# UMEssen/Body-and-Organ-Analysis

Measured on AMD Instinct MI355X. Metric: CT volumes/sec (512^3 @1.5 mm, total+bca) on MI355X, higher is better.
Workload: dtype f16

## Files before the change

### body-and-organ-analysis_amd/boa_hip/_lib.py

```python
from __future__ import annotations

import ctypes as C
import os

_HERE = os.path.dirname(os.path.abspath(__file__))
LIB_PATH = os.environ.get("BOA_HIP_LIB") or os.path.join(_HERE, "libboa_hip.so")

BOA_OK, BOA_EINVAL, BOA_EHIP, BOA_ENOMEM, BOA_EINF = 0, -1, -2, -3, -4
BOA_DEFLATE_DYNAMIC = 1
BOA_INF_INFO_WORDS, BOA_INF_MS_WORDS = 8, 8
BOA_INF_STATUS = ("ok", "truncated", "invalid", "far", "overrun", "size", "crc", "repair", "trailing")
BOA_PLAN_WORDS = 32
K_CONV_MFMA, K_CONV_FIRST, K_CONVT, K_NORM_FINALIZE, K_HEAD_ACCUM, K_ARGMAX, K_OTHER, K_AGG, K_MORPH, K_RESAMPLE, K_COPY, K_COUNT = range(12)
K_NAMES = ["conv_mfma", "conv_first", "convT_mfma", "norm_finalize", "head_accum", "finalize_argmax", "other", "aggregation",
           "morphology", "resample", "copy_remap"]
CNT_NAMES = ["head_mfma", "head_valu", "conv_ws", "conv_simple", "first_mfma", "first_valu", "f32", "conv_x3", "x3", "head_gather",
             "copy_t", "bbox_vec", "finalize_vec8"]
MAX_STAGES = 8


class NetDesc(C.Structure):
    _fields_ = [
        ("n_stages", C.c_int), ("in_channels", C.c_int), ("num_classes", C.c_int),
        ("features", C.c_int * MAX_STAGES), ("kernel", (C.c_int * 3) * MAX_STAGES),
        ("stride", (C.c_int * 3) * MAX_STAGES), ("n_conv_enc", C.c_int * MAX_STAGES),
        ("n_conv_dec", C.c_int * MAX_STAGES), ("patch", C.c_int * 3), ("norm_eps", C.c_float),
        ("lrelu_slope", C.c_float),
    ]


class BoaError(RuntimeError):
    pass


_lib = None

vp, i32, u64, f32 = C.c_void_p, C.c_int, C.c_size_t, C.c_float
ip = C.POINTER(C.c_int)

_PROTOS = {
    "boa_last_error": (C.c_char_p, []),
    "boa_version": (i32, []),
    "boa_init": (i32, [i32, vp, C.POINTER(vp)]),
    "boa_destroy": (None, [vp]),
    "boa_device_info": (i32, [vp, C.c_char_p, i32, ip, C.POINTER(u64), C.POINTER(u64)]),
    "boa_malloc": (i32, [vp, u64, C.POINTER(vp)]),
    "boa_free": (i32, [vp, vp]),
    "boa_trim": (i32, [vp]),
    "boa_bind_thread": (i32, [vp]),
    "boa_host_alloc": (i32, [vp, C.c_size_t, C.POINTER(vp)]),
    "boa_host_free": (i32, [vp, vp]),
    "boa_mfma_peak": (i32, [vp, i32, i32, C.POINTER(C.c_double)]),
    "boa_memset": (i32, [vp, vp, i32, u64]),
    "boa_h2d": (i32, [vp, vp, vp, u64]),
    "boa_d2h": (i32, [vp, vp, vp, u64]),
    "boa_sync": (i32, [vp]),
    "boa_timer_start": (i32, [vp, i32]),
    "boa_timer_stop": (i32, [vp, i32, C.POINTER(f32)]),
    "boa_prof_enable": (i32, [vp, i32]),
    "boa_prof_reset": (i32, [vp]),
    "boa_prof_get": (i32, [vp, i32, C.POINTER(C.c_double), C.POINTER(C.c_longlong), C.POINTER(C.c_double),
                           C.POINTER(C.c_double)]),
    "boa_debug_counter": (C.c_longlong, [vp, i32, i32]),
    "boa_net_debug_activation": (i32, [vp, i32, i32, i32, i32, vp, ip, ip]),
    "boa_net_debug_layer": (i32, [vp, i32, i32, i32, i32, vp, vp, vp, ip, ip, ip]),
    "boa_head_tile": (i32, [vp, vp, vp, i32, ip, i32, vp, vp, f32, vp, vp, vp, vp, ip, ip]),
    "boa_head_tile_f32": (i32, [vp, i32, vp, u64, vp, i32, ip, i32, vp, vp, f32, vp, vp, vp, vp, ip, ip]),
    "boa_ct_normalize": (i32, [vp, vp, i32, vp, u64, f32, f32, f32, f32]),
    "boa_accumulate_tile": (i32, [vp, vp, vp, vp, vp, i32, ip, ip, ip]),
    "boa_finalize_labels": (i32, [vp, vp, vp, i32, ip, vp, i32, i32, i32, vp, i32, vp, ip, ip, vp]),
    "boa_finalize_labels_planes": (i32, [vp, vp, vp, i32, ip, vp, i32, i32, i32, vp, i32, vp, ip, ip, vp, i32, i32]),
    "boa_net_predict_sliding_window_deferred": (i32, [vp, vp, ip, ip, ip, ip, i32, vp, vp, vp, ip, C.POINTER(vp)]),
    "boa_net_apply_deferred": (i32, [vp, vp, vp, vp, vp, ip]),
    "boa_stash_destroy": (None, [vp]),
    "boa_net_create": (i32, [vp, C.POINTER(NetDesc), vp, u64, i32, i32, C.POINTER(vp)]),
    "boa_net_destroy": (None, [vp]),
    "boa_net_weight_count": (u64, [C.POINTER(NetDesc)]),
    "boa_net_load_weights": (i32, [vp, vp, u64]),
    "boa_net_set_mirroring": (i32, [vp, i32]),
    "boa_net_forward": (i32, [vp, vp, ip, ip, i32, vp]),
    "boa_net_predict_sliding_window": (i32, [vp, vp, ip, ip, ip, ip, i32, vp, vp, vp]),
    "boa_net_labels_supported": (i32, [vp, ip, i32]),
    "boa_net_predict_labels_fold": (i32, [vp, vp, ip, ip, ip, ip, i32, vp, vp, i32, i32, vp, i32, vp, ip, ip, vp]),
    "boa_conv_block_test": (i32, [vp, vp, i32, i32, ip, vp, vp, vp, vp, i32, ip, ip, i32, i32, vp]),
    "boa_convtranspose_test": (i32, [vp, vp, i32, i32, ip, vp, vp, i32, ip, vp]),
    "boa_conv_plan": (i32, [i32, i32, ip, i32, ip, ip, i32, i32, ip, ip]),
    "boa_convt_plan": (i32, [i32, ip, i32, ip, i32, i32, i32, ip]),
    "boa_conv_layer_test": (i32, [vp, i32, i32, ip, vp, i32, vp, vp, vp, i32, vp, vp, vp, vp, vp, vp, i32, ip, ip, ip, vp, vp, vp, vp, ip]),
    "boa_convt_layer_test": (i32, [vp, i32, i32, ip, vp, i32, vp, vp, vp, vp, i32, ip, vp, ip]),
    "boa_tissue_aggregate": (i32, [vp, vp, vp, vp, vp, vp, i32, i32, i32, vp, vp]),
    "boa_slice_label_presence": (i32, [vp, vp, i32, i32, i32, vp]),
    "boa_tissue_projections": (i32, [vp, vp, vp, i32, i32, i32, vp, i32, vp, vp, vp, vp]),
    "boa_label_hu_histogram": (i32, [vp, vp, vp, vp, u64, i32, i32, vp]),
    "boa_label_hu_mask": (i32, [vp, vp, vp, vp, i32, i32, i32, u64, vp]),
    "boa_label_basic_stats": (i32, [vp, vp, i32, vp, ip, i32, vp]),
    "boa_label_apply_lut": (i32, [vp, vp, u64, vp, vp]),
    "boa_group_stats_f64": (i32, [vp, vp, vp, u64, vp, i32, vp, vp]),
    "boa_label_hu_mask_f64": (i32, [vp, vp, vp, vp, i32, C.c_double, C.c_double, u64, vp]),
    "boa_tissue_aggregate_f64": (i32, [vp, vp, vp, vp, vp, vp, i32, i32, i32, vp, vp]),
    "boa_binary_erode": (i32, [vp, vp, vp, vp, i32, i32, i32, i32]),
    "boa_ccl26": (i32, [vp, vp, i32, i32, i32, vp, vp, ip]),
    "boa_ccl_filter_largest": (i32, [vp, vp, vp, u64, vp, i32]),
    "boa_ccl_remove_small": (i32, [vp, vp, vp, u64, C.c_uint32, vp]),
    "boa_ccl_list_components": (i32, [vp, vp, u64, i32, vp, vp, ip]),
    "boa_scatter_u32": (i32, [vp, vp, vp, vp, i32]),
    "boa_ccl_fill_unmarked": (i32, [vp, vp, vp, u64, C.c_uint32, vp, i32]),
    "boa_label_blobs6": (i32, [vp, vp, i32, i32, i32, vp, vp, ip]),
    "boa_label_blobs_filter": (i32, [vp, vp, vp, u64, vp, C.c_uint32, C.c_uint32, vp]),
    "boa_label_select": (i32, [vp, vp, u64, i32, ip, vp]),
    "boa_fill_holes_2d": (i32, [vp, vp, i32, i32, i32, vp, vp, vp]),
    "boa_binary_dilate_cross": (i32, [vp, vp, vp, vp, i32, i32, i32, i32]),
    "boa_mask_assign": (i32, [vp, vp, u64, i32, i32, vp]),
    "boa_label_overlay": (i32, [vp, vp, u64, vp]),
    "boa_median3_inplane": (i32, [vp, vp, i32, i32, i32, i32, vp]),
    "boa_median3_inplane_f64": (i32, [vp, vp, i32, i32, i32, i32, vp]),
    "boa_bits_words": (u64, [i32, i32, i32]),
    "boa_bits_erode_u8": (i32, [vp, vp, vp, i32, i32, i32, i32, i32]),
    "boa_bits_select": (i32, [vp, vp, i32, i32, i32, vp, i32, vp]),
    "boa_bits_unpack": (i32, [vp, vp, i32, i32, i32, vp]),
    "boa_bits_fill_supported": (i32, [i32, i32]),
    "boa_bits_fill_holes_2d": (i32, [vp, vp, i32, i32, i32, i32, vp]),
    "boa_bits_remove_small": (i32, [vp, vp, i32, i32, i32, i32, C.c_uint32, i32]),
    "boa_bits_filter_largest": (i32, [vp, vp, i32, i32, i32, vp, i32]),
    "boa_bits_assign_labels": (i32, [vp, vp, i32, i32, i32, i32, vp, vp]),
    "boa_copy3": (i32, [vp, vp, i32, C.c_longlong, C.POINTER(C.c_longlong), ip, vp, i32, C.c_longlong, C.POINTER(C.c_longlong)]),
    "boa_nonzero_bbox": (i32, [vp, vp, i32, ip, ip]),
    "boa_resample_cubic": (i32, [vp, vp, i32, ip, vp, i32, ip]),
    "boa_resample_nearest_u8": (i32, [vp, vp, ip, vp, ip]),
    "boa_resample_onehot_u8": (i32, [vp, vp, ip, vp, ip, i32]),
    "boa_resize_skimage_f32": (i32, [vp, vp, ip, vp, ip, i32, i32]),
    "boa_resize_logits_argmax": (i32, [vp, vp, i32, ip, ip, ip, ip, i32, vp, i32, vp]),
    "boa_logits_to_probabilities": (i32, [vp, vp, i32, ip, ip, ip, ip, i32, ip, ip, ip, vp, vp, vp]),
    "boa_comm_available": (i32, []),
    "boa_comm_library": (C.c_char_p, []),
    "boa_comm_unique_id": (i32, [vp]),
    "boa_comm_create": (i32, [vp, i32, i32, vp, C.POINTER(vp)]),
    "boa_comm_destroy": (None, [vp]),
    "boa_comm_wait": (i32, [vp]),
    "boa_comm_exchange": (i32, [vp, i32, C.POINTER(vp), C.POINTER(u64), i32, i32, C.POINTER(vp), C.POINTER(u64), i32]),
    "boa_comm_shift_slab": (i32, [vp, i32, i32, i32, i32, i32, i32, vp, vp, i32, ip, vp]),
    "boa_comm_all_reduce": (i32, [vp, vp, u64, i32]),
    "boa_comm_planes_to_owner": (i32, [vp, vp, i32, ip, i32, ip, ip, ip, i32, ip, ip, ip]),
    "boa_comm_stats": (i32, [vp, C.POINTER(C.c_longlong), C.POINTER(C.c_longlong)]),
    "boa_add_f16_planes": (i32, [vp, vp, vp, vp, i32, ip, i32, i32]),
    "boa_ljpeg_decode": (i32, [vp, vp, u64, i32, ip, i32, ip, i32, ip, i32, C.POINTER(C.c_uint32), vp, ip, i32]),
    "boa_jdct_decode": (i32, [vp, vp, u64, i32, ip, i32, i32, i32, ip, i32, ip, i32, C.POINTER(C.c_uint32), i32,
                        C.POINTER(C.c_uint16), vp, ip, i32]),
    "boa_j2k_decode": (i32, [vp, vp, u64, i32, ip, i32, ip, vp, ip]),
    "boa_rle_decode": (i32, [vp, vp, u64, i32, ip, i32, i32, i32, vp, ip, i32]),
    "boa_jls_decode": (i32, [vp, vp, u64, i32, ip, i32, i32, vp, ip, i32]),
    "boa_deflate_bound": (u64, [u64, u64]),
    "boa_deflate_members": (i32, [vp, vp, u64, u64, i32, vp, u64, C.POINTER(u64), C.POINTER(C.c_uint32)]),
    "boa_deflate_members2": (i32, [vp, vp, u64, u64, i32, i32, i32, vp, u64, C.POINTER(u64), C.POINTER(C.c_uint32)]),
    "boa_label_member_presence": (i32, [vp, vp, u64, u64, C.POINTER(C.c_uint32)]),
    "boa_deflate_label_pairs": (i32, [vp, vp, u64, u64, i32, i32, C.POINTER(C.c_uint8), C.POINTER(C.c_uint32), i32, vp, u64, C.POINTER(u64),
                                      C.POINTER(C.c_uint32)]),
    "boa_inflate_default_chunk": (u64, []),
    "boa_inflate_streams": (i32, [vp, vp, u64, i32, C.POINTER(u64), C.POINTER(u64), C.POINTER(u64), C.POINTER(C.c_uint32), u64, vp, u64, ip,
                                  C.POINTER(u64), C.POINTER(C.c_float)]),
}

EXPORTS = sorted(_PROTOS)


def lib():
    global _lib
    if _lib is not None:
        return _lib
    if not os.path.exists(LIB_PATH):
        raise BoaError(
            f"{LIB_PATH} not found: build it with `make -C body-and-organ-analysis_amd` "
            "(or python -c 'import __graft_entry__ as g; g.build()'). There is no CPU fallback.")
    try:
        import torch
    except Exception:
        pass
    L = C.CDLL(LIB_PATH, mode=C.RTLD_GLOBAL)
    for name, (res, args) in _PROTOS.items():
        fn = getattr(L, name)
        fn.restype = res
        fn.argtypes = args
    _lib = L
    return L


def check(rc: int, what: str = ""):
    if rc == BOA_OK:
        return
    msg = lib().boa_last_error().decode("utf-8", "replace")
    text = f"{what}: {msg}" if what else msg
    if rc == BOA_EINVAL:
        raise ValueError(text)
    if rc == BOA_ENOMEM:
        raise MemoryError(text)
    raise BoaError(text)


def int3(v):
    return (C.c_int * 3)(*[int(x) for x in v])
```

### body-and-organ-analysis_amd/boa_hip/resample.py

```python
from __future__ import annotations

import numpy as np

from ._lib import check, int3
from .device import Context, DeviceBuffer

_IN_DTYPES = {np.dtype(np.int16): 0, np.dtype(np.float32): 1, np.dtype(np.float64): 2, np.dtype(np.int32): 3}


def zoomed_shape(shape, zoom):
    zoom = np.broadcast_to(np.asarray(zoom, dtype=np.float64), (len(shape),))
    return tuple(int(round(n * z)) for n, z in zip(shape, zoom))


def resample_cubic_device(ctx: Context, dev_in: DeviceBuffer, in_dtype, in_shape, out_shape, out_dtype=np.int32):
    code = _IN_DTYPES[np.dtype(in_dtype)]
    oc = {np.dtype(np.int32): 0, np.dtype(np.float64): 1}[np.dtype(out_dtype)]
    n = int(np.prod(out_shape))
    out = DeviceBuffer(ctx, n * np.dtype(out_dtype).itemsize)
    check(ctx.lib.boa_resample_cubic(ctx.h, dev_in.vp, code, int3(in_shape), out.vp, oc, int3(out_shape)),
          "boa_resample_cubic")
    return out


def resample_nearest_device(ctx: Context, dev_in: DeviceBuffer, in_shape, out_shape):
    out = DeviceBuffer(ctx, int(np.prod(out_shape)))
    check(ctx.lib.boa_resample_nearest_u8(ctx.h, dev_in.vp, int3(in_shape), out.vp, int3(out_shape)),
          "boa_resample_nearest_u8")
    return out


REF_TO_MEMORY_AXIS = (2, 0, 1)


def resample_onehot_device(ctx: Context, dev_in: DeviceBuffer, in_shape, out_shape, sep_axis=None):
    out = DeviceBuffer(ctx, int(np.prod(out_shape)))
    ax = -1 if sep_axis is None or int(sep_axis) < 0 else REF_TO_MEMORY_AXIS[int(sep_axis)]
    check(ctx.lib.boa_resample_onehot_u8(ctx.h, dev_in.vp, int3(in_shape), out.vp, int3(out_shape), ax),
          "boa_resample_onehot_u8")
    return out


def resample_img(ctx: Context, img: np.ndarray, zoom=0.5, order: int = 0, out_dtype=None, target_shape=None):
    img = np.asarray(img)
    if img.ndim != 3:
        raise ValueError(f"resample_img: 3-D arrays only, got {img.shape}")
    shape = tuple(int(s) for s in target_shape) if target_shape is not None else zoomed_shape(img.shape, zoom)
    if order == 0:
        if img.dtype != np.uint8:
            if img.min() < 0 or img.max() > 255:
                raise ValueError("resample_img(order=0): label values must fit uint8")
            img = img.astype(np.uint8)
        d = DeviceBuffer(ctx, img.size).upload(img)
        o = resample_nearest_device(ctx, d, img.shape, shape)
        res = o.download(shape, np.uint8)
        d.free(), o.free()
        return res
    if order != 3:
        raise ValueError(f"resample_img: order {order} not supported (the reference uses 0 and 3)")
    if img.dtype not in _IN_DTYPES:
        img = img.astype(np.float64)
    od = np.dtype(np.float64 if out_dtype is None else out_dtype)
    d = DeviceBuffer(ctx, img.nbytes).upload(img)
    o = resample_cubic_device(ctx, d, img.dtype, img.shape, shape, od)
    res = o.download(shape, od)
    d.free(), o.free()
    return res


def change_spacing_array(ctx: Context, data: np.ndarray, img_spacing, new_spacing=1.25, target_shape=None, order=0,
                         dtype=None, remove_negative=False):
    old_shape = np.array(data.shape)
    img_spacing = np.array(img_spacing, dtype=np.float32)
    if target_shape is not None:
        zoom = np.array(target_shape) / old_shape
        new_spacing = img_spacing / zoom
    else:
        if type(new_spacing) is float:
            new_spacing = [new_spacing] * 3
        new_spacing = np.array(new_spacing)
        zoom = img_spacing / new_spacing
    if np.array_equal(img_spacing, new_spacing):
        return data, None
    want_i32 = dtype is not None and np.dtype(dtype) == np.int32 and not remove_negative and order == 3
    new = resample_img(ctx, data, zoom, order, out_dtype=np.int32 if want_i32 else None)
    if remove_negative:
        new[new < 1e-4] = 0
    if dtype is not None:
        new = new.astype(dtype, copy=False)
    return new, zoom


def new_affine(affine: np.ndarray, zoom) -> np.ndarray:
    a = np.copy(affine)
    for i in range(3):
        a[:3, i] = a[:3, i] / zoom[i]
    return a
```

### body-and-organ-analysis_amd/csrc/resample.hip

```cpp
#include <math.h>

#include "common.h"
#include "resample_logits.h"

#define NPAD 12

template <typename T>
__global__ __launch_bounds__(256) void k_pad_edge_f64(const T* __restrict__ in, int X, int Y, int Z,
                                                      double* __restrict__ out) {
    const int PX = X + 2 * NPAD, PY = Y + 2 * NPAD, PZ = Z + 2 * NPAD;
    const size_t n = (size_t)PX * PY * PZ;
    size_t i = (size_t)blockIdx.x * 256 + threadIdx.x;
    if (i >= n) return;
    int x, y, z;
    idx3(i, PY, PZ, x, y, z);
    x -= NPAD; y -= NPAD; z -= NPAD;
    x = min(max(x, 0), X - 1);
    y = min(max(y, 0), Y - 1);
    z = min(max(z, 0), Z - 1);
    out[i] = (double)in[((size_t)x * Y + y) * Z + z];
}

struct SplineConsts {
    double z, gain, z_n, init_scale, tail_scale;
};

__global__ __launch_bounds__(64) void k_spline_filter_axis(double* __restrict__ c, int n, size_t st, int n1, size_t st1,
                                                           int n2, size_t st2, SplineConsts k) {
    const size_t line = (size_t)blockIdx.x * 64 + threadIdx.x;
    if (line >= (size_t)n1 * n2) return;
    double* p = c + (line / n2) * st1 + (line % n2) * st2;
    const double z = k.z;
    const double gain = k.gain;
    for (int i = 0; i < n; ++i) p[i * st] *= gain;
    const double z_n = k.z_n;
    double z_i = z;
    const double c0 = p[0];
    double acc = p[0] + z_n * p[(size_t)(n - 1) * st];
    for (int i = 1; i < n; ++i) {
        acc += z_i * (p[i * st] + z_n * p[(size_t)(n - 1 - i) * st]);
        z_i *= z;
    }
    acc *= k.init_scale;
    acc += c0;
    p[0] = acc;
    for (int i = 1; i < n; ++i) p[i * st] += z * p[(size_t)(i - 1) * st];
    p[(size_t)(n - 1) * st] *= k.tail_scale;
    for (int i = n - 2; i >= 0; --i) p[i * st] = z * (p[(size_t)(i + 1) * st] - p[i * st]);
}

__global__ __launch_bounds__(64) void k_spline_filter_contig(double* __restrict__ c, int n, int n1, size_t st1, int n2, size_t st2,
                                                             SplineConsts k) {
    const size_t line = (size_t)blockIdx.x * 64 + threadIdx.x;
    if (line >= (size_t)n1 * n2) return;
    double* p = c + (line / n2) * st1 + (line % n2) * st2;
    const double z = k.z, gain = k.gain, z_n = k.z_n;
    const int nc = n / 8;
    const double c0 = p[0] * gain;
    double acc = c0 + z_n * (p[n - 1] * gain);
    double z_i = z;
    for (int cb = 0; cb < nc; ++cb) {
        double f[8], b[8];
#pragma unroll
        for (int m = 0; m < 8; ++m) f[m] = p[8 * cb + m];
        const int b0 = n - 8 * cb - 8;
#pragma unroll
        for (int m = 0; m < 8; ++m) b[m] = p[b0 + m];
#pragma unroll
        for (int m = 0; m < 8; ++m) {
            const int i = 8 * cb + m;
            if (i >= 1) {
                acc += z_i * (f[m] * gain + z_n * (b[7 - m] * gain));
                z_i *= z;
            }
        }
    }
    for (int i = max(8 * nc, 1); i < n; ++i) {
        acc += z_i * (p[i] * gain + z_n * (p[n - 1 - i] * gain));
        z_i *= z;
    }
    acc *= k.init_scale;
    acc += c0;
    double prev = acc;
    for (int cb = 0; cb < nc; ++cb) {
        double f[8];
#pragma unroll
        for (int m = 0; m < 8; ++m) f[m] = p[8 * cb + m];
#pragma unroll
        for (int m = 0; m < 8; ++m) {
            if (8 * cb + m >= 1) {
                double s = f[m] * gain;
                s += z * prev;
                prev = s;
            }
            f[m] = prev;
        }
#pragma unroll
        for (int m = 0; m < 8; ++m) p[8 * cb + m] = f[m];
    }
    for (int i = 8 * nc; i < n; ++i) {
        if (i >= 1) {
            double s = p[i] * gain;
            s += z * prev;
            prev = s;
        }
        p[i] = prev;
    }
    double nxt = p[n - 1] * k.tail_scale;
    p[n - 1] = nxt;
    int i = n - 2;
    for (; i >= 0 && ((i + 1) & 7) != 0; --i) {
        nxt = z * (nxt - p[i]);
        p[i] = nxt;
    }
    for (; i >= 7; i -= 8) {
        double f[8];
#pragma unroll
        for (int m = 0; m < 8; ++m) f[m] = p[i - 7 + m];
#pragma unroll
        for (int m = 7; m >= 0; --m) {
            nxt = z * (nxt - f[m]);
            f[m] = nxt;
        }
#pragma unroll
        for (int m = 0; m < 8; ++m) p[i - 7 + m] = f[m];
    }
}

__device__ __forceinline__ void cubic_weights(double cc, int* start, double w[4]) {
    const double fl = floor(cc);
    const double x = cc - fl;
    const double y = x, zz = 1.0 - x;
    w[1] = (y * y * (y - 2.0) * 3.0 + 4.0) / 6.0;
    w[2] = (zz * zz * (zz - 2.0) * 3.0 + 4.0) / 6.0;
    w[0] = zz * zz * zz / 6.0;
    w[3] = 1.0 - w[0] - w[1] - w[2];
    *start = (int)fl - 1;
}

__global__ __launch_bounds__(256) void k_zoom_cubic(const double* __restrict__ coef, int X, int Y, int Z, int OX, int OY,
                                                    int OZ, double zx, double zy, double zz_, int out_mode, void* out) {
    const size_t n = (size_t)OX * OY * OZ;
    size_t i = (size_t)blockIdx.x * 256 + threadIdx.x;
    if (i >= n) return;
    int ox, oy, oz;
    idx3(i, OY, OZ, ox, oy, oz);
    const int PY = Y + 2 * NPAD, PZ = Z + 2 * NPAD;
    double wx[4], wy[4], wz[4];
    int sx, sy, sz;
    cubic_weights((double)ox * zx + NPAD, &sx, wx);
    cubic_weights((double)oy * zy + NPAD, &sy, wy);
    cubic_weights((double)oz * zz_ + NPAD, &sz, wz);
    double t = 0.0;
#pragma unroll
    for (int a = 0; a < 4; ++a)
#pragma unroll
        for (int b = 0; b < 4; ++b) {
            const double* row = coef + ((size_t)(sx + a) * PY + (sy + b)) * PZ + sz;
#pragma unroll
            for (int d = 0; d < 4; ++d) {
                double cf = row[d];
                cf *= wx[a];
                cf *= wy[b];
                cf *= wz[d];
                t += cf;
            }
        }
    if (out_mode == 0)
        ((int*)out)[i] = (int)t;
    else
        ((double*)out)[i] = t;
}

__global__ __launch_bounds__(256) void k_zoom_nearest_u8(const unsigned char* __restrict__ in, int X, int Y, int Z, int OX,
                                                         int OY, int OZ, double zx, double zy, double zz_,
                                                         unsigned char* __restrict__ out) {
    const size_t n = (size_t)OX * OY * OZ;
    size_t i = (size_t)blockIdx.x * 256 + threadIdx.x;
    if (i >= n) return;
    int ox, oy, oz;
    idx3(i, OY, OZ, ox, oy, oz);
    const int ix = min(max((int)floor((double)ox * zx + 0.5), 0), X - 1);
    const int iy = min(max((int)floor((double)oy * zy + 0.5), 0), Y - 1);
    const int iz = min(max((int)floor((double)oz * zz_ + 0.5), 0), Z - 1);
    out[i] = in[((size_t)ix * Y + iy) * Z + iz];
}

static SplineConsts spline_consts(int n) {
    SplineConsts k;
    k.z = -0x1.126145e9ecd56p-2;
    k.gain = (1.0 - 1.0 / k.z) * (1.0 - k.z);
    k.z_n = pow(k.z, (double)n);
    k.init_scale = k.z / (1.0 - k.z_n * k.z_n);
    k.tail_scale = k.z / (k.z - 1.0);
    return k;
}

static double zoom_factor(int n_in, int n_out) { return n_out > 1 ? (double)(n_in - 1) / (double)(n_out - 1) : 1.0; }

extern "C" int boa_resample_cubic(boa_ctx* c, const void* dev_in, int in_dtype, const int in_dims[3], void* dev_out,
                                  int out_dtype, const int out_dims[3]) {
    BOA_REQUIRE(c && dev_in && dev_out && in_dims && out_dims, "boa_resample_cubic: NULL argument");
    BOA_REQUIRE(in_dtype >= 0 && in_dtype <= 3, "boa_resample_cubic: in_dtype %d (0 int16, 1 float32, 2 float64, 3 int32)", in_dtype);
    BOA_REQUIRE(out_dtype == 0 || out_dtype == 1, "boa_resample_cubic: out_dtype %d (0 int32, 1 float64)", out_dtype);
    const int X = in_dims[0], Y = in_dims[1], Z = in_dims[2];
    for (int a = 0; a < 3; ++a) BOA_REQUIRE(in_dims[a] >= 2 && out_dims[a] >= 1, "boa_resample_cubic: bad dims");
    const int PX = X + 2 * NPAD, PY = Y + 2 * NPAD, PZ = Z + 2 * NPAD;
    const size_t pn = (size_t)PX * PY * PZ;
    double* coef = nullptr;
    BOA_TRY(boa_malloc(c, pn * sizeof(double), (void**)&coef));
    const unsigned gp = (unsigned)((pn + 255) / 256);
    KernelTimer t(c, BOA_K_RESAMPLE, 0, (double)pn * 8.0 * 8);
    switch (in_dtype) {
        case 0: hipLaunchKernelGGL(k_pad_edge_f64<short>, dim3(gp), dim3(256), 0, c->stream, (const short*)dev_in, X, Y, Z, coef); break;
        case 1: hipLaunchKernelGGL(k_pad_edge_f64<float>, dim3(gp), dim3(256), 0, c->stream, (const float*)dev_in, X, Y, Z, coef); break;
        case 2: hipLaunchKernelGGL(k_pad_edge_f64<double>, dim3(gp), dim3(256), 0, c->stream, (const double*)dev_in, X, Y, Z, coef); break;
        default: hipLaunchKernelGGL(k_pad_edge_f64<int>, dim3(gp), dim3(256), 0, c->stream, (const int*)dev_in, X, Y, Z, coef); break;
    }
    hipLaunchKernelGGL(k_spline_filter_axis, dim3((unsigned)(((size_t)PY * PZ + 63) / 64)), dim3(64), 0, c->stream, coef, PX,
                       (size_t)PY * PZ, PY, (size_t)PZ, PZ, (size_t)1, spline_consts(PX));
    hipLaunchKernelGGL(k_spline_filter_axis, dim3((unsigned)(((size_t)PX * PZ + 63) / 64)), dim3(64), 0, c->stream, coef, PY,
                       (size_t)PZ, PX, (size_t)PY * PZ, PZ, (size_t)1, spline_consts(PY));
    hipLaunchKernelGGL(k_spline_filter_contig, dim3((unsigned)(((size_t)PX * PY + 63) / 64)), dim3(64), 0, c->stream, coef, PZ, PX,
                       (size_t)PY * PZ, PY, (size_t)PZ, spline_consts(PZ));
    const size_t on = (size_t)out_dims[0] * out_dims[1] * out_dims[2];
    hipLaunchKernelGGL(k_zoom_cubic, dim3((unsigned)((on + 255) / 256)), dim3(256), 0, c->stream, coef, X, Y, Z, out_dims[0],
                       out_dims[1], out_dims[2], zoom_factor(X, out_dims[0]), zoom_factor(Y, out_dims[1]),
                       zoom_factor(Z, out_dims[2]), out_dtype, dev_out);
    t.stop();
    hipError_t e = hipGetLastError();
    int rc = boa_free(c, coef);
    BOA_HIP_TRY(e);
    return rc;
}

extern "C" int boa_resample_nearest_u8(boa_ctx* c, const uint8_t* dev_in, const int in_dims[3], uint8_t* dev_out,
                                       const int out_dims[3]) {
    BOA_REQUIRE(c && dev_in && dev_out && in_dims && out_dims, "boa_resample_nearest_u8: NULL argument");
    for (int a = 0; a < 3; ++a) BOA_REQUIRE(in_dims[a] >= 1 && out_dims[a] >= 1, "boa_resample_nearest_u8: bad dims");
    const size_t on = (size_t)out_dims[0] * out_dims[1] * out_dims[2];
    KernelTimer t(c, BOA_K_RESAMPLE, 0, (double)on * 2.0);
    hipLaunchKernelGGL(k_zoom_nearest_u8, dim3((unsigned)((on + 255) / 256)), dim3(256), 0, c->stream, dev_in, in_dims[0],
                       in_dims[1], in_dims[2], out_dims[0], out_dims[1], out_dims[2], zoom_factor(in_dims[0], out_dims[0]),
                       zoom_factor(in_dims[1], out_dims[1]), zoom_factor(in_dims[2], out_dims[2]), dev_out);
    t.stop();
    BOA_HIP_TRY(hipGetLastError());
    return BOA_OK;
}



__device__ __forceinline__ unsigned f2ord(float f) {
    const unsigned u = __float_as_uint(f);
    return (u & 0x80000000u) ? ~u : (u | 0x80000000u);
}
__device__ __forceinline__ float ord2f(unsigned u) { return __uint_as_float((u & 0x80000000u) ? (u & 0x7fffffffu) : ~u); }

__global__ __launch_bounds__(256) void k_minmax_groups(const float* __restrict__ in, int X, int Y, int Z, int gaxis,
                                                       unsigned* __restrict__ mm ) {
    const size_t n = (size_t)X * Y * Z;
    const size_t i0 = ((size_t)blockIdx.x * 256 + threadIdx.x) * 8;
    if (i0 >= n) return;
    int cur = -1;
    float lo = 0.f, hi = 0.f;
    for (int k = 0; k < 8 && i0 + k < n; ++k) {
        const size_t i = i0 + k;
        const int z = (int)(i % Z), y = (int)((i / Z) % Y), x = (int)(i / ((size_t)Z * Y));
        const int g = gaxis < 0 ? 0 : (gaxis == 0 ? x : (gaxis == 1 ? y : z));
        const float v = in[i];
        if (g != cur) {
            if (cur >= 0) {
                atomicMin(&mm[2 * cur], f2ord(lo));
                atomicMax(&mm[2 * cur + 1], f2ord(hi));
            }
            cur = g;
            lo = hi = v;
        } else {
            lo = fminf(lo, v);
            hi = fmaxf(hi, v);
        }
    }
    if (cur >= 0) {
        atomicMin(&mm[2 * cur], f2ord(lo));
        atomicMax(&mm[2 * cur + 1], f2ord(hi));
    }
}

__global__ __launch_bounds__(256) void k_pad_edge_axes_f64(const float* __restrict__ in, int X, int Y, int Z, int px, int py, int pz,
                                                           double* __restrict__ out) {
    const int PX = X + 2 * px, PY = Y + 2 * py, PZ = Z + 2 * pz;
    const size_t n = (size_t)PX * PY * PZ;
    size_t i = (size_t)blockIdx.x * 256 + threadIdx.x;
    if (i >= n) return;
    int x, y, z;
    idx3(i, PY, PZ, x, y, z);
    x -= px; y -= py; z -= pz;
    x = min(max(x, 0), X - 1);
    y = min(max(y, 0), Y - 1);
    z = min(max(z, 0), Z - 1);
    out[i] = (double)in[((size_t)x * Y + y) * Z + z];
}

struct ResizeArgs {
    int I[3], P[3], O[3];
    int act[3];
    double zf[3];
    int gaxis;
};

__global__ __launch_bounds__(256) void k_resize_cubic_f32(const double* __restrict__ coef, ResizeArgs a, const unsigned* __restrict__ mm,
                                                          float* __restrict__ out) {
    const size_t n = (size_t)a.O[0] * a.O[1] * a.O[2];
    size_t i = (size_t)blockIdx.x * 256 + threadIdx.x;
    if (i >= n) return;
    int o[3];
    idx3(i, a.O[1], a.O[2], o[0], o[1], o[2]);
    double w[3][4];
    int st[3], nt[3];
#pragma unroll
    for (int d = 0; d < 3; ++d) {
        if (a.act[d]) {
            cubic_weights(((double)o[d] + 0.5) * a.zf[d] - 0.5 + NPAD, &st[d], w[d]);
            nt[d] = 4;
        } else {
            st[d] = a.I[d] == a.O[d] ? o[d] : nearest_src(o[d], a.zf[d], a.I[d]);
            nt[d] = 1;
        }
    }
    double t = 0.0;
    for (int p = 0; p < nt[0]; ++p)
        for (int q = 0; q < nt[1]; ++q) {
            const double* row = coef + ((size_t)(st[0] + p) * a.P[1] + (st[1] + q)) * a.P[2] + st[2];
            for (int r = 0; r < nt[2]; ++r) {
                double cf = row[r];
                if (a.act[0]) cf *= w[0][p];
                if (a.act[1]) cf *= w[1][q];
                if (a.act[2]) cf *= w[2][r];
                t += cf;
            }
        }
    const int g = a.gaxis < 0 ? 0 : st[a.gaxis];
    const double lo = (double)ord2f(mm[2 * g]), hi = (double)ord2f(mm[2 * g + 1]);
    t = t < lo ? lo : (t > hi ? hi : t);
    out[i] = (float)t;
}

struct LogitsResizeArgs {
    LogitsResizeGeom g;
    int merge;
    unsigned char lut[256];
};

__global__ __launch_bounds__(256) void k_resize_logits_argmax(LogitsResizeArgs a, unsigned char* __restrict__ labels) {
    const size_t n = (size_t)a.g.O[0] * a.g.O[1] * a.g.O[2];
    size_t i = (size_t)blockIdx.x * 256 + threadIdx.x;
    if (i >= n) return;
    int o[3];
    idx3(i, a.g.O[1], a.g.O[2], o[0], o[1], o[2]);
    LogitsTaps t;
    logits_taps(a.g, o, t);
    float best = 0.f;
    int bidx = 0;
    bool bnan = false;
    for (int c = 0; c < a.g.C; ++c) {
        const float f = us2f(logits_resampled(a.g, t, c));
        const bool isn = f != f;
        if (c == 0) {
            best = f;
            bnan = isn;
        } else if (!bnan && (isn || f > best)) {
            best = f;
            bidx = c;
            bnan = isn;
        }
    }
    if (a.merge) {
        if (bidx != 0) labels[i] = a.lut[bidx];
    } else {
// ... 89 lines not shown
```

### include/boa_hip.h

```cpp
#ifndef BOA_HIP_H
#define BOA_HIP_H

#include <stddef.h>
#include <stdint.h>

#ifdef __cplusplus
extern "C" {
#endif

#define BOA_OK 0
#define BOA_EINVAL (-1)
#define BOA_EHIP (-2)
#define BOA_ENOMEM (-3)
#define BOA_EINF (-4)

typedef struct boa_ctx boa_ctx;
typedef struct boa_net boa_net;

const char* boa_last_error(void);
int boa_version(void);
int boa_init(int device, void* stream, boa_ctx** out);
void boa_destroy(boa_ctx* ctx);
int boa_device_info(boa_ctx* ctx, char* name, int name_len, int* cu_count, size_t* total_mem, size_t* free_mem);
int boa_malloc(boa_ctx* ctx, size_t bytes, void** dev_out);
// ... 70 lines not shown
    float lrelu_slope;
} boa_net_desc;

int boa_net_create(boa_ctx* ctx, const boa_net_desc* desc, const float* host_weights, size_t n_floats,
                   int max_batch, int precision, boa_net** out);
void boa_net_destroy(boa_net* net);
size_t boa_net_weight_count(const boa_net_desc* desc);
int boa_net_load_weights(boa_net* net, const float* host_weights, size_t n_floats);

int boa_net_set_mirroring(boa_net* net, int axes_mask);

int boa_net_forward(boa_net* net, const float* dev_volume, const int V[3], const int* host_origins,
                    int n_tiles, float* dev_logits_out);

int boa_net_predict_sliding_window(boa_net* net, const float* dev_volume, const int V[3], const int PV[3],
                                   const int* vol_off, const int* host_origins, int n_tiles,
                                   const uint16_t* dev_gauss, uint16_t* dev_acc, uint16_t* dev_n);

int boa_net_labels_supported(boa_net* net, const int* host_origins, int n_tiles);
int boa_net_predict_labels_fold(boa_net* net, const float* dev_volume, const int V[3], const int PV[3], const int* vol_off,
                                const int* host_origins, int n_tiles, const uint16_t* dev_gauss, uint16_t* dev_fold,
                                int fold_index, int n_folds, const uint8_t* host_lut, int merge, uint8_t* dev_labels_out,
                                const int* crop_off, const int* crop_dims, int* dev_inf_flag);

typedef struct boa_stash boa_stash;
int boa_net_predict_sliding_window_deferred(boa_net* net, const float* dev_volume, const int V[3], const int PV[3],
                                            const int* vol_off, const int* host_origins, int n_tiles,
                                            const uint16_t* dev_gauss, uint16_t* dev_acc, uint16_t* dev_n,
                                            const int* host_defer_planes, boa_stash** stash_out);
int boa_net_apply_deferred(boa_net* net, const boa_stash* stash, const uint16_t* dev_gauss, uint16_t* dev_acc,
                           uint16_t* dev_n, const int PV[3]);
void boa_stash_destroy(boa_stash* stash);

int boa_conv_block_test(boa_ctx* ctx, const float* dev_in, int N, int Cin, const int dims[3],
                        const float* host_w, const float* host_b, const float* host_gamma, const float* host_beta,
                        int Cout, const int kernel[3], const int stride[3], int with_norm_act, int impl,
                        float* dev_out);
int boa_net_debug_activation(boa_net* net, int kind, int stage, int conv, int tile, float* dev_out, int* channels_out,
                             int dims_out[3]);
#define BOA_LK_FIRST_VALU 1
#define BOA_LK_FIRST_MFMA 2
#define BOA_LK_CONV_WS 3
#define BOA_LK_CONV_NS 4
#define BOA_LK_CONV_MFMA 5
#define BOA_LK_CONV_F32 6
#define BOA_LK_CONVT_X3 7
#define BOA_LK_CONVT_MFMA 8
#define BOA_LK_CONVT_RW 9
#define BOA_LK_CONVT_DEEP 10
#define BOA_LK_CONVT_F32 11
#define BOA_LK_HEAD_X3 12
#define BOA_LK_HEAD_F32 13
#define BOA_LK_HEAD_MFMA 14
int boa_net_debug_layer(boa_net* net, int kind, int stage, int conv, int tile, float* dev_raw, float* host_ss, uint16_t* host_ss16,
                        int* channels_out, int dims_out[3], int* host_info);

int boa_head_tile(boa_ctx* ctx, const uint16_t* dev_act, const float* dev_ss, int F0, const int P[3], int C,
                  const float* dev_w, const float* dev_b, float slope, float* dev_logits_out, const uint16_t* dev_gauss,
                  uint16_t* dev_acc, uint16_t* dev_n, const int PV[3], const int start[3]);
int boa_head_tile_f32(boa_ctx* ctx, int kind, const float* dev_act_f32, size_t stride, const float* dev_ss, int F0, const int P[3], int C,
                      const float* dev_w, const float* dev_b, float slope, float* dev_logits_out, const uint16_t* dev_gauss,
                      uint16_t* dev_acc, uint16_t* dev_n, const int PV[3], const int start[3]);
int boa_convtranspose_test(boa_ctx* ctx, const float* dev_in, int N, int Cin, const int dims[3],
                           const float* host_w, const float* host_b, int Cout, const int stride[3], float* dev_out);

#define BOA_PLAN_WORDS 32
int boa_conv_plan(int Cin0, int Cin1, const int dims[3], int Cout, const int kernel[3], const int stride[3], int cu_count, int mode,
                  const int* plan_override, int* plan_out);
int boa_convt_plan(int Cin, const int dims[3], int Cout, const int stride[3], int cu_count, int mode, int norm_src, int* plan_out);
int boa_conv_layer_test(boa_ctx* ctx, int mode, int N, const int dims[3], const float* dev_src0, int C0, const float* dev_ss0,
                        const uint32_t* dev_ss16_0, const float* dev_src1, int C1, const float* dev_ss1, const uint32_t* dev_ss16_1,
                        const float* host_w, const float* host_b, const float* host_gamma, const float* host_beta, int Cout,
                        const int kernel[3], const int stride[3], const int* plan_override, void* dev_raw, float* dev_ss,
                        uint32_t* dev_ss16, float* dev_partials, int* host_plan);
int boa_convt_layer_test(boa_ctx* ctx, int mode, int N, const int dims[3], const float* dev_src, int Cin, const float* dev_ss,
                         const uint32_t* dev_ss16, const float* host_w, const float* host_b, int Cout, const int stride[3], void* dev_raw,
                         int* host_plan);

int boa_tissue_aggregate(boa_ctx* ctx, const int16_t* dev_ct, const int16_t* dev_ct_rules, const uint8_t* dev_regions,
                         const uint8_t* dev_parts,
                         uint8_t* dev_tissues_out, int Z, int Y, int X, uint32_t* dev_counts, int64_t* dev_hu_sums);

int boa_slice_label_presence(boa_ctx* ctx, const uint8_t* dev_labels, int Z, int Y, int X, uint8_t* dev_present);

int boa_tissue_projections(boa_ctx* ctx, const uint8_t* dev_tissues, const uint8_t* dev_regions, int Z, int Y, int X,
                           const uint8_t* host_values, int n_values, uint32_t* dev_coronal, uint32_t* dev_sagittal,
                           uint8_t* dev_mask_coronal, uint8_t* dev_mask_sagittal);

int boa_label_hu_histogram(boa_ctx* ctx, const int16_t* dev_ct, const uint8_t* dev_labels, const uint8_t* dev_mask,
                           size_t n_voxels, int hu_min, int nbins, uint32_t* dev_hist);

int boa_label_hu_mask(boa_ctx* ctx, const int16_t* dev_ct, const uint8_t* dev_labels, const uint8_t* host_lut,
                      int mode, int hu_lo, int hu_hi, size_t n_voxels, uint8_t* dev_mask_out);

#define BOA_LABEL_STATS_WORDS 770
int boa_label_basic_stats(boa_ctx* ctx, const void* dev_ct, int ct_dtype, const uint8_t* dev_labels, const int dims[3], int border,
                          uint64_t* dev_out);
int boa_label_apply_lut(boa_ctx* ctx, const uint8_t* dev_labels, size_t n, const uint8_t host_lut[256], uint8_t* dev_out);

#define BOA_GROUP_STATS_F64_COLS 10
int boa_group_stats_f64(boa_ctx* ctx, const double* dev_ct, const uint8_t* dev_labels, size_t n_voxels, const uint8_t* host_lut,
                        int n_groups, uint64_t* host_count, double* host_stats);
int boa_label_hu_mask_f64(boa_ctx* ctx, const double* dev_ct, const uint8_t* dev_labels, const uint8_t* host_lut,
                          int mode, double hu_lo, double hu_hi, size_t n_voxels, uint8_t* dev_mask_out);
int boa_tissue_aggregate_f64(boa_ctx* ctx, const double* dev_ct, const double* dev_ct_rules, const uint8_t* dev_regions,
                             const uint8_t* dev_parts, uint8_t* dev_tissues_out, int Z, int Y, int X, uint32_t* dev_counts,
                             double* dev_hu_sums);

int boa_binary_erode(boa_ctx* ctx, const uint8_t* dev_mask, uint8_t* dev_out, uint8_t* dev_tmp, int Z, int Y, int X,
                     int kernel_value);

int boa_ccl26(boa_ctx* ctx, const uint8_t* dev_mask, int Z, int Y, int X, int32_t* dev_roots, uint32_t* dev_sizes,
              int* host_n_components);
int boa_ccl_filter_largest(boa_ctx* ctx, const int32_t* dev_roots, const uint32_t* dev_sizes, size_t n,
                           uint8_t* dev_seg, int fill_value);
int boa_ccl_remove_small(boa_ctx* ctx, const int32_t* dev_roots, const uint32_t* dev_sizes, size_t n,
                         uint32_t max_size, uint8_t* dev_mask_inout);
int boa_ccl_list_components(boa_ctx* ctx, const uint32_t* dev_sizes, size_t n, int max_out, int32_t* host_roots,
                            uint32_t* host_sizes, int* host_count);
int boa_scatter_u32(boa_ctx* ctx, uint32_t* dev_dst, const int32_t* host_idx, const uint32_t* host_val, int m);
int boa_ccl_fill_unmarked(boa_ctx* ctx, const int32_t* dev_roots, const uint32_t* dev_sizes, size_t n, uint32_t mark,
                          uint8_t* dev_seg, int fill_value);
int boa_label_blobs6(boa_ctx* ctx, const uint8_t* dev_labels, int D0, int D1, int D2, int32_t* dev_roots, uint32_t* dev_sizes,
                     int* host_n_components);
int boa_label_blobs_filter(boa_ctx* ctx, const int32_t* dev_roots, const uint32_t* dev_sizes, size_t n, const uint8_t host_mode[256],
                           uint32_t lo, uint32_t hi, uint8_t* dev_labels_inout);
int boa_label_select(boa_ctx* ctx, const uint8_t* dev_labels, size_t n, int mode, const int vals[3],
                     uint8_t* dev_mask_out);

int boa_fill_holes_2d(boa_ctx* ctx, const uint8_t* dev_mask, int Z, int Y, int X, int32_t* dev_scratch_i32,
                      uint8_t* dev_scratch_u8, uint8_t* dev_out);
int boa_binary_dilate_cross(boa_ctx* ctx, const uint8_t* dev_mask, uint8_t* dev_out, uint8_t* dev_tmp, int Z, int Y, int X,
                            int iterations);
int boa_mask_assign(boa_ctx* ctx, const uint8_t* dev_mask, size_t n, int invert, int value, uint8_t* dev_out);
size_t boa_bits_words(int Z, int Y, int X);
int boa_bits_erode_u8(boa_ctx* ctx, const uint8_t* dev_mask, uint8_t* dev_out, int Z, int Y, int X, int lo, int hi);
int boa_bits_select(boa_ctx* ctx, const uint8_t* dev_seg, int Z, int Y, int X, const uint8_t host_lut[256], int n_masks, uint32_t* dev_bits);
int boa_bits_unpack(boa_ctx* ctx, const uint32_t* dev_bits, int Z, int Y, int X, uint8_t* dev_out);
int boa_bits_fill_supported(int Y, int X);
int boa_bits_fill_holes_2d(boa_ctx* ctx, const uint32_t* dev_in, int Z, int Y, int X, int n_masks, uint32_t* dev_out);
int boa_bits_remove_small(boa_ctx* ctx, uint32_t* dev_bits, int Z, int Y, int X, int n_masks, uint32_t max_size, int invert);
int boa_bits_filter_largest(boa_ctx* ctx, const uint32_t* dev_bits, int Z, int Y, int X, uint8_t* dev_seg, int fill_value);
int boa_bits_assign_labels(boa_ctx* ctx, const uint32_t* dev_bits, int Z, int Y, int X, int n_masks, const uint8_t* host_labels, uint8_t* dev_out);
int boa_label_overlay(boa_ctx* ctx, const uint8_t* dev_part, size_t n, uint8_t* dev_out);
int boa_median3_inplane(boa_ctx* ctx, const int16_t* dev_in, int Z, int Y, int X, int flat_axis, int16_t* dev_out);
int boa_median3_inplane_f64(boa_ctx* ctx, const double* dev_in, int Z, int Y, int X, int flat_axis, double* dev_out);

int boa_copy3(boa_ctx* ctx, const void* dev_in, int in_dtype, long long in_off, const long long in_step[3],
              const int dims[3], void* dev_out, int out_dtype, long long out_off, const long long out_step[3]);
int boa_nonzero_bbox(boa_ctx* ctx, const void* dev_in, int dtype, const int dims[3], int host_bbox[6]);

int boa_resample_cubic(boa_ctx* ctx, const void* dev_in, int in_dtype, const int in_dims[3], void* dev_out, int out_dtype,
                       const int out_dims[3]);
int boa_resample_nearest_u8(boa_ctx* ctx, const uint8_t* dev_in, const int in_dims[3], uint8_t* dev_out,
                            const int out_dims[3]);
int boa_resample_onehot_u8(boa_ctx* ctx, const uint8_t* dev_in, const int in_dims[3], uint8_t* dev_out, const int out_dims[3],
                           int sep_axis);


int boa_resize_skimage_f32(boa_ctx* ctx, const float* dev_in, const int in_dims[3], float* dev_out, const int out_dims[3],
                           int order, int slice_axis);
int boa_resize_logits_argmax(boa_ctx* ctx, const uint16_t* dev_logits, int C, const int grid_dims[3], const int* crop_off,
                             const int* crop_dims, const int out_dims[3], int slice_axis, const uint8_t* host_lut, int merge,
                             uint8_t* dev_labels_out);

int boa_logits_to_probabilities(boa_ctx* ctx, const uint16_t* dev_logits, int C, const int grid_dims[3], const int* crop_off,
                                const int* crop_dims, const int* out_dims, int slice_axis, const int bbox_lo[3],
                                const int full_dims[3], const int perm[3], float* dev_prob, const uint8_t* host_lut,
                                uint8_t* dev_labels);

typedef struct boa_comm boa_comm;
int boa_comm_available(void);
const char* boa_comm_library(void);
int boa_comm_unique_id(unsigned char id_out[128]);
int boa_comm_create(boa_ctx* ctx, int world, int rank, const unsigned char id[128], boa_comm** out);
void boa_comm_destroy(boa_comm* comm);
int boa_comm_wait(boa_comm* comm);
int boa_comm_exchange(boa_comm* comm, int dst, const void* const* send_ptrs, const size_t* send_bytes, int n_send, int src,
                      void* const* recv_ptrs, const size_t* recv_bytes, int n_recv);
int boa_comm_shift_slab(boa_comm* comm, int dst, int send_lo, int send_hi, int src, int recv_lo, int recv_hi, uint16_t* dev_acc,
                        uint16_t* dev_n, int C, const int PV[3], uint16_t* recv_stage);
int boa_comm_all_reduce(boa_comm* comm, void* dev, size_t count, int dtype);
int boa_comm_planes_to_owner(boa_comm* comm, uint16_t* dev_logits, int C, const int PV[3], int n_send, const int* send_peer,
                             const int* send_lo, const int* send_hi, int n_recv, const int* recv_peer, const int* recv_lo,
                             const int* recv_hi);
int boa_comm_stats(boa_comm* comm, long long* calls, long long* bytes);
int boa_add_f16_planes(boa_ctx* ctx, uint16_t* dev_acc, uint16_t* dev_n, const uint16_t* dev_stage, int C, const int PV[3], int lo, int hi);

#define BOA_LJ_FRAME_WORDS 16
#define BOA_LJ_F_OFF_LO 0
#define BOA_LJ_F_OFF_HI 1
#define BOA_LJ_F_LEN 2
#define BOA_LJ_F_ROWS 3
#define BOA_LJ_F_COLS 4
#define BOA_LJ_F_P 5
#define BOA_LJ_F_PT 6
#define BOA_LJ_F_PRED 7
#define BOA_LJ_F_RESTART_ROWS 8
#define BOA_LJ_F_TABLE 9
#define BOA_LJ_F_SEG_FIRST 10
#define BOA_LJ_F_N_SEG 11
#define BOA_LJ_F_SUB_FIRST 12
#define BOA_LJ_F_N_SUB 13
#define BOA_LJ_TABLE_WORDS 384
#define BOA_LJ_OK 0
#define BOA_LJ_TRUNCATED 1
#define BOA_LJ_INVALID_CODE 2
#define BOA_LJ_TRAILING_GARBAGE 3
int boa_ljpeg_decode(boa_ctx* ctx, const uint8_t* dev_data, size_t data_bytes, int n_frames, const int* frames, int n_segs,
                     const int* segs, int n_subs, const int* subs, int n_tables, const uint32_t* tables, uint16_t* dev_out,
                     int* host_status, int serial);

#define BOA_JD_FRAME_WORDS 16
#define BOA_JD_F_OFF_LO 0
#define BOA_JD_F_OFF_HI 1
#define BOA_JD_F_LEN 2
#define BOA_JD_F_P 3
#define BOA_JD_F_RESTART 4
#define BOA_JD_F_DC_TABLE 5
#define BOA_JD_F_AC_TABLE 6
#define BOA_JD_F_QTABLE 7
#define BOA_JD_F_SEG_FIRST 8
#define BOA_JD_F_N_SEG 9
#define BOA_JD_F_SUB_FIRST 10
#define BOA_JD_F_N_SUB 11
#define BOA_JD_OK 0
#define BOA_JD_TRUNCATED 1
#define BOA_JD_INVALID_CODE 2
#define BOA_JD_RUN_PAST_BLOCK 3
#define BOA_JD_BAD_SSSS 4
#define BOA_JD_TRAILING 5
int boa_jdct_decode(boa_ctx* ctx, const uint8_t* dev_data, size_t data_bytes, int n_frames, const int* frames, int rows, int cols,
                    int n_segs, const int* segs, int n_subs, const int* subs, int n_tables, const uint32_t* tables, int n_qtables,
                    const uint16_t* qtables, uint16_t* dev_out, int* host_status, int serial);

#define BOA_J2K_FRAME_WORDS 12
#define BOA_J2K_F_OUT_LO 0
#define BOA_J2K_F_OUT_HI 1
#define BOA_J2K_F_ROWS 2
#define BOA_J2K_F_COLS 3
#define BOA_J2K_F_LEVELS 4
#define BOA_J2K_F_P 5
#define BOA_J2K_F_SIGNED 6
#define BOA_J2K_F_BLOCK_FIRST 7
#define BOA_J2K_F_N_BLOCKS 8
#define BOA_J2K_F_TRANSFORM 9
#define BOA_J2K_T_97 0
#define BOA_J2K_T_53 1
#define BOA_J2K_BLOCK_WORDS 12
#define BOA_J2K_B_FRAME 0
#define BOA_J2K_B_ORIENT 1
#define BOA_J2K_B_X0 2
#define BOA_J2K_B_Y0 3
#define BOA_J2K_B_W 4
#define BOA_J2K_B_H 5
#define BOA_J2K_B_NUMBPS 6
#define BOA_J2K_B_PASSES 7
#define BOA_J2K_B_OFF_LO 8
#define BOA_J2K_B_OFF_HI 9
#define BOA_J2K_B_LEN 10
#define BOA_J2K_B_STEP 11
#define BOA_J2K_OK 0
#define BOA_J2K_INVALID 1
int boa_j2k_decode(boa_ctx* ctx, const uint8_t* dev_data, size_t data_bytes, int n_frames, const int* frames, int n_blocks,
                   const int* blocks, uint16_t* dev_out, int* host_status);

#define BOA_RLE_FRAME_WORDS 8
#define BOA_RLE_F_OFF_LO 0
#define BOA_RLE_F_OFF_HI 1
#define BOA_RLE_F_LEN 2
#define BOA_RLE_F_N_SEG 3
#define BOA_RLE_F_SEG 4
#define BOA_RLE_OK 0
#define BOA_RLE_TRUNCATED 1
int boa_rle_decode(boa_ctx* ctx, const uint8_t* dev_data, size_t data_bytes, int n_frames, const int* frames, int rows, int cols,
                   int chunk_bytes, uint16_t* dev_out, int* host_status, int serial);

#define BOA_JLS_FRAME_WORDS 16
#define BOA_JLS_F_OFF_LO 0
#define BOA_JLS_F_OFF_HI 1
#define BOA_JLS_F_LEN 2
#define BOA_JLS_F_MAXVAL 3
#define BOA_JLS_F_NEAR 4
#define BOA_JLS_F_T1 5
#define BOA_JLS_F_T2 6
#define BOA_JLS_F_T3 7
#define BOA_JLS_F_RESET 8
#define BOA_JLS_WAVE_MAX_COLS 4096
#define BOA_JLS_OK 0
#define BOA_JLS_TRUNCATED 1
#define BOA_JLS_INVALID 2
int boa_jls_decode(boa_ctx* ctx, const uint8_t* dev_data, size_t data_bytes, int n_frames, const int* frames, int rows, int cols,
                   uint16_t* dev_out, int* host_status, int serial);

size_t boa_deflate_bound(size_t n, size_t member_bytes);
int boa_deflate_members(boa_ctx* ctx, const uint8_t* dev_src, size_t n, size_t member_bytes, int row_bytes, uint8_t* dev_out,
                        size_t out_capacity, size_t* host_offsets, uint32_t* host_crc32);
#define BOA_DEFLATE_DYNAMIC 1
int boa_deflate_members2(boa_ctx* ctx, const uint8_t* dev_src, size_t n, size_t member_bytes, int row_bytes, int near_bytes, int flags,
                         uint8_t* dev_out, size_t out_capacity, size_t* host_offsets, uint32_t* host_crc32);

int boa_label_member_presence(boa_ctx* ctx, const uint8_t* dev_labels, size_t n, size_t member_bytes, uint32_t* host_bits);
int boa_deflate_label_pairs(boa_ctx* ctx, const uint8_t* dev_labels, size_t n, size_t member_bytes, int row_bytes, int flags,
                            const uint8_t* host_pair_label, const uint32_t* host_pair_member, int n_pairs, uint8_t* dev_out,
                            size_t out_capacity, size_t* host_offsets, uint32_t* host_crc32);

// ... 31 lines not shown
```

Baseline: 0.5939.

## Add LDS-staged spline prefilter path for int16 cubic resample along last axis

Adds a cubic resample path for int16 inputs where only the last axis is rescaled. Each B-spline prefilter pass stages several lines in LDS, with cooperative coalesced loads and stores around a per-line recursive filter. The first pass fuses the int16-to-double conversion and edge padding into the load. The goal is to avoid strided global-memory recursion and the separate padding/convert passes, at the cost of fewer parallel threads during the filter step and high LDS use per block.

```diff
diff --git a/body-and-organ-analysis_amd/boa_hip/_lib.py b/body-and-organ-analysis_amd/boa_hip/_lib.py
--- a/body-and-organ-analysis_amd/boa_hip/_lib.py
+++ b/body-and-organ-analysis_amd/boa_hip/_lib.py
@@ -126,6 +126,8 @@
     "boa_copy3": (i32, [vp, vp, i32, C.c_longlong, C.POINTER(C.c_longlong), ip, vp, i32, C.c_longlong, C.POINTER(C.c_longlong)]),
     "boa_nonzero_bbox": (i32, [vp, vp, i32, ip, ip]),
     "boa_resample_cubic": (i32, [vp, vp, i32, ip, vp, i32, ip]),
+    "boa_resample_cubic_axis2_supported": (i32, [ip]),
+    "boa_resample_cubic_axis2": (i32, [vp, vp, ip, vp, i32, ip]),
     "boa_resample_nearest_u8": (i32, [vp, vp, ip, vp, ip]),
     "boa_resample_onehot_u8": (i32, [vp, vp, ip, vp, ip, i32]),
     "boa_resize_skimage_f32": (i32, [vp, vp, ip, vp, ip, i32, i32]),
diff --git a/body-and-organ-analysis_amd/boa_hip/resample.py b/body-and-organ-analysis_amd/boa_hip/resample.py
--- a/body-and-organ-analysis_amd/boa_hip/resample.py
+++ b/body-and-organ-analysis_amd/boa_hip/resample.py
@@ -13,13 +13,25 @@
     return tuple(int(round(n * z)) for n, z in zip(shape, zoom))
 
 
-def resample_cubic_device(ctx: Context, dev_in: DeviceBuffer, in_dtype, in_shape, out_shape, out_dtype=np.int32):
+def cubic_path(ctx: Context, in_dtype, in_shape, out_shape) -> str:
+    rescaled = [int(a) != int(b) for a, b in zip(in_shape, out_shape)]
+    if np.dtype(in_dtype) == np.int16 and rescaled == [False, False, True] \
+            and ctx.lib.boa_resample_cubic_axis2_supported(int3(in_shape)):
+        return "axis2"
+    return "three_pass"
+
+
+def resample_cubic_device(ctx: Context, dev_in: DeviceBuffer, in_dtype, in_shape, out_shape, out_dtype=np.int32, path=None):
     code = _IN_DTYPES[np.dtype(in_dtype)]
     oc = {np.dtype(np.int32): 0, np.dtype(np.float64): 1}[np.dtype(out_dtype)]
     n = int(np.prod(out_shape))
     out = DeviceBuffer(ctx, n * np.dtype(out_dtype).itemsize)
-    check(ctx.lib.boa_resample_cubic(ctx.h, dev_in.vp, code, int3(in_shape), out.vp, oc, int3(out_shape)),
-          "boa_resample_cubic")
+    if (path or cubic_path(ctx, in_dtype, in_shape, out_shape)) == "axis2":
+        check(ctx.lib.boa_resample_cubic_axis2(ctx.h, dev_in.vp, int3(in_shape), out.vp, oc, int3(out_shape)),
+              "boa_resample_cubic_axis2")
+    else:
+        check(ctx.lib.boa_resample_cubic(ctx.h, dev_in.vp, code, int3(in_shape), out.vp, oc, int3(out_shape)),
+              "boa_resample_cubic")
     return out
 
 
diff --git a/body-and-organ-analysis_amd/csrc/resample.hip b/body-and-organ-analysis_amd/csrc/resample.hip
--- a/body-and-organ-analysis_amd/csrc/resample.hip
+++ b/body-and-organ-analysis_amd/csrc/resample.hip
@@ -49,11 +49,7 @@
     for (int i = n - 2; i >= 0; --i) p[i * st] = z * (p[(size_t)(i + 1) * st] - p[i * st]);
 }
 
-__global__ __launch_bounds__(64) void k_spline_filter_contig(double* __restrict__ c, int n, int n1, size_t st1, int n2, size_t st2,
-                                                             SplineConsts k) {
-    const size_t line = (size_t)blockIdx.x * 64 + threadIdx.x;
-    if (line >= (size_t)n1 * n2) return;
-    double* p = c + (line / n2) * st1 + (line % n2) * st2;
+__device__ __forceinline__ void spline_line_contig(double* p, int n, const SplineConsts& k) {
     const double z = k.z, gain = k.gain, z_n = k.z_n;
     const int nc = n / 8;
     const double c0 = p[0] * gain;
@@ -125,6 +121,13 @@
 #pragma unroll
         for (int m = 0; m < 8; ++m) p[i - 7 + m] = f[m];
     }
+}
+
+__global__ __launch_bounds__(64) void k_spline_filter_contig(double* __restrict__ c, int n, int n1, size_t st1, int n2, size_t st2,
+                                                             SplineConsts k) {
+    const size_t line = (size_t)blockIdx.x * 64 + threadIdx.x;
+    if (line >= (size_t)n1 * n2) return;
+    spline_line_contig(c + (line / n2) * st1 + (line % n2) * st2, n, k);
 }
 
 __device__ __forceinline__ void cubic_weights(double cc, int* start, double w[4]) {
@@ -224,6 +227,117 @@
     hipLaunchKernelGGL(k_spline_filter_contig, dim3((unsigned)(((size_t)PX * PY + 63) / 64)), dim3(64), 0, c->stream, coef, PZ, PX,
                        (size_t)PY * PZ, PY, (size_t)PZ, spline_consts(PZ));
     const size_t on = (size_t)out_dims[0] * out_dims[1] * out_dims[2];
+    hipLaunchKernelGGL(k_zoom_cubic, dim3((unsigned)((on + 255) / 256)), dim3(256), 0, c->stream, coef, X, Y, Z, out_dims[0],
+                       out_dims[1], out_dims[2], zoom_factor(X, out_dims[0]), zoom_factor(Y, out_dims[1]),
+                       zoom_factor(Z, out_dims[2]), out_dtype, dev_out);
+    t.stop();
+    hipError_t e = hipGetLastError();
+    int rc = boa_free(c, coef);
+    BOA_HIP_TRY(e);
+    return rc;
+}
+
+#define SL_LINES 16
+#define SL_LDS_MAX (72 * 1024)
+
+struct SplineLines {
+    int n, n_real;
+    int n2;
+    size_t nlines;
+    size_t src_st, src_st1, src_st2;
+    size_t dst_st, dst_st1, dst_st2;
+    int lane_lines;
+    int L, ls;
+};
+
+template <typename T>
+__global__ __launch_bounds__(256) void k_spline_lines_lds(const T* src, double* dst, SplineLines a, SplineConsts k) {
+    extern __shared__ double sl_buf[];
+    __shared__ size_t sl_src[SL_LINES], sl_dst[SL_LINES];
+    const size_t line0 = (size_t)blockIdx.x * a.L;
+    const int nl = (int)min((size_t)a.L, a.nlines - line0);
+    const int t = threadIdx.x;
+    if (t < nl) {
+        const size_t line = line0 + t, q = line / a.n2, r = line % a.n2;
+        sl_src[t] = q * a.src_st1 + r * a.src_st2;
+        sl_dst[t] = q * a.dst_st1 + r * a.dst_st2;
+    }
+    __syncthreads();
+    const int l0 = a.lane_lines ? (t & (a.L - 1)) : (t >> 6), dl = a.lane_lines ? a.L : 4;
+    const int i0 = a.lane_lines ? t / a.L : (t & 63), di = a.lane_lines ? 256 / a.L : 64;
+    for (int l = l0; l < nl; l += dl) {
+        const T* s = src + sl_src[l];
+        double* b = sl_buf + l * a.ls;
+        for (int i = i0; i < a.n; i += di) b[i] = (double)s[(size_t)min(max(i - NPAD, 0), a.n_real - 1) * a.src_st];
+    }
+    __syncthreads();
+    if (t < nl) spline_line_contig(sl_buf + t * a.ls, a.n, k);
+    __syncthreads();
+    for (int l = l0; l < nl; l += dl) {
+        double* d = dst + sl_dst[l];
+        const double* b = sl_buf + l * a.ls;
+        for (int i = i0; i < a.n; i += di) d[(size_t)i * a.dst_st] = b[i];
+    }
+}
+
+static bool spline_lines_plan(int n, SplineLines* a) {
+    a->ls = n | 1;
+    a->L = SL_LINES;
+    while (a->L >= 1 && (size_t)a->L * a->ls * sizeof(double) > SL_LDS_MAX) a->L /= 2;
+    return a->L >= 1;
+}
+
+template <typename T>
+static void launch_spline_lines(boa_ctx* c, const T* src, double* dst, const SplineLines& a) {
+    static bool once = (hipFuncSetAttribute((const void*)k_spline_lines_lds<T>, hipFuncAttributeMaxDynamicSharedMemorySize, SL_LDS_MAX), true);
+    (void)once;
+    hipLaunchKernelGGL(k_spline_lines_lds<T>, dim3((unsigned)((a.nlines + a.L - 1) / a.L)), dim3(256), (size_t)a.L * a.ls * sizeof(double),
+                       c->stream, src, dst, a, spline_consts(a.n));
+}
+
+extern "C" int boa_resample_cubic_axis2_supported(const int in_dims[3]) {
+    if (!in_dims) return 0;
+    SplineLines a;
+    for (int d = 0; d < 3; ++d)
+        if (in_dims[d] < 2 || !spline_lines_plan(in_dims[d] + 2 * NPAD, &a)) return 0;
+    const size_t gmax = (size_t)1 << 31;
+    if ((size_t)in_dims[1] * in_dims[2] >= gmax || (size_t)(in_dims[0] + 2 * NPAD) * in_dims[2] >= gmax) return 0;
+    return(size_t)(in_dims[0] + 2 * NPAD) * (in_dims[1] + 2 * NPAD) < ((size_t)1 << 31) * SL_LINES ? 1 : 0;
+}
+
+extern "C" int boa_resample_cubic_axis2(boa_ctx* c, const int16_t* dev_in, const int in_dims[3], void* dev_out, int out_dtype,
+                                        const int out_dims[3]) {
+    BOA_REQUIRE(c && dev_in && dev_out && in_dims && out_dims, "boa_resample_cubic_axis2: NULL argument");
+    BOA_REQUIRE(out_dtype == 0 || out_dtype == 1, "boa_resample_cubic_axis2: out_dtype %d (0 int32, 1 float64)", out_dtype);
+    BOA_REQUIRE(out_dims[0] == in_dims[0] && out_dims[1] == in_dims[1] && out_dims[2] >= 1,
+                "boa_resample_cubic_axis2: only the last axis may be rescaled (in %d x %d x %d, out %d x %d x %d)", in_dims[0], in_dims[1],
+                in_dims[2], out_dims[0], out_dims[1], out_dims[2]);
+    BOA_REQUIRE(boa_resample_cubic_axis2_supported(in_dims), "boa_resample_cubic_axis2: dims %d x %d x %d not supported", in_dims[0],
+                in_dims[1], in_dims[2]);
+    const int X = in_dims[0], Y = in_dims[1], Z = in_dims[2];
+    const int PX = X + 2 * NPAD, PY = Y + 2 * NPAD, PZ = Z + 2 * NPAD;
+    const size_t pn = (size_t)PX * PY * PZ, s0 = (size_t)PY * PZ, s1 = (size_t)PZ;
+    double* coef = nullptr;
+    BOA_TRY(boa_malloc(c, pn * sizeof(double), (void**)&coef));
+    const size_t on = (size_t)out_dims[0] * out_dims[1] * out_dims[2];
+    KernelTimer t(c, BOA_K_RESAMPLE, 0, (double)X * Y * Z * 2.0 + (double)pn * 8.0 * 6 + (double)on * (out_dtype ? 8.0 : 4.0));
+    double* real = coef + NPAD * s1 + NPAD;
+    SplineLines a;
+    spline_lines_plan(PX, &a);
+    a.n = PX; a.n_real = X; a.n2 = Z; a.nlines = (size_t)Y * Z; a.lane_lines = 1;
+    a.src_st = (size_t)Y * Z; a.src_st1 = (size_t)Z; a.src_st2 = 1;
+    a.dst_st = s0; a.dst_st1 = s1; a.dst_st2 = 1;
+    launch_spline_lines<short>(c, dev_in, real, a);
+    spline_lines_plan(PY, &a);
+    a.n = PY; a.n_real = Y; a.n2 = Z; a.nlines = (size_t)PX * Z; a.lane_lines = 1;
+    a.src_st = s1; a.src_st1 = s0; a.src_st2 = 1;
+    a.dst_st = s1; a.dst_st1 = s0; a.dst_st2 = 1;
+    launch_spline_lines<double>(c, real, coef + NPAD, a);
+    spline_lines_plan(PZ, &a);
+    a.n = PZ; a.n_real = Z; a.n2 = PY; a.nlines = (size_t)PX * PY; a.lane_lines = 0;
+    a.src_st = 1; a.src_st1 = s0; a.src_st2 = s1;
+    a.dst_st = 1; a.dst_st1 = s0; a.dst_st2 = s1;
+    launch_spline_lines<double>(c, coef + NPAD, coef, a);
     hipLaunchKernelGGL(k_zoom_cubic, dim3((unsigned)((on + 255) / 256)), dim3(256), 0, c->stream, coef, X, Y, Z, out_dims[0],
                        out_dims[1], out_dims[2], zoom_factor(X, out_dims[0]), zoom_factor(Y, out_dims[1]),
                        zoom_factor(Z, out_dims[2]), out_dtype, dev_out);
diff --git a/include/boa_hip.h b/include/boa_hip.h
--- a/include/boa_hip.h
+++ b/include/boa_hip.h
@@ -246,6 +246,9 @@
 
 int boa_resample_cubic(boa_ctx* ctx, const void* dev_in, int in_dtype, const int in_dims[3], void* dev_out, int out_dtype,
                        const int out_dims[3]);
+int boa_resample_cubic_axis2_supported(const int in_dims[3]);
+int boa_resample_cubic_axis2(boa_ctx* ctx, const int16_t* dev_in, const int in_dims[3], void* dev_out, int out_dtype,
+                             const int out_dims[3]);
 int boa_resample_nearest_u8(boa_ctx* ctx, const uint8_t* dev_in, const int in_dims[3], uint8_t* dev_out,
                             const int out_dims[3]);
 int boa_resample_onehot_u8(boa_ctx* ctx, const uint8_t* dev_in, const int in_dims[3], uint8_t* dev_out, const int out_dims[3],
```

Result: no change. 0.5939 (median of 2 runs) (+0.0%).
